# endernewton/tf-faster-rcnn

Hardware: NVIDIA H100
Metric: images/sec (higher is better)
Workload: dtype f16x3 (fp32-grade: fp16 hi/lo split of both operands, 3 wgmma f16 MMAs per product, fp32 accumulate)

## Files before the change

### include/frcnn_b200.h

```cpp
#ifndef FRCNN_B200_H_
#define FRCNN_B200_H_

#include <stddef.h>
#include <stdint.h>

#ifdef __cplusplus
extern "C" {
#endif

typedef enum {
  FRCNN_OK = 0,
  FRCNN_ERR_CUDA = -1,
  FRCNN_ERR_ARG = -2,
  FRCNN_ERR_NO_DEVICE = -3,
  FRCNN_ERR_DRIVER_ENTRY = -4,
  FRCNN_ERR_CAPACITY = -5
} frcnn_status;

#define FRCNN_NMS_PLUS_ONE 1u
#define FRCNN_NMS_INCLUSIVE 2u
#define FRCNN_NMS_SKIP_DEGENERATE 4u
#define FRCNN_NMS_MODE_CPU_NMS (FRCNN_NMS_PLUS_ONE | FRCNN_NMS_INCLUSIVE)
#define FRCNN_NMS_MODE_GPU_NMS (FRCNN_NMS_PLUS_ONE)
#define FRCNN_NMS_MODE_TF (FRCNN_NMS_SKIP_DEGENERATE)

#define FRCNN_ACT_NONE 0
#define FRCNN_ACT_RELU 1
#define FRCNN_ACT_RELU6 2

int frcnn_version(void);
int frcnn_last_error(char* buf, size_t buflen);
int frcnn_check_device(int device_id);
int frcnn_zero_async(void* dev_ptr, size_t bytes, void* stream);

typedef struct frcnn_graph frcnn_graph;
int frcnn_graph_begin(void* stream);
int frcnn_graph_end(void* stream, frcnn_graph** out);
int frcnn_graph_launch(const frcnn_graph* g, void* stream);
void frcnn_graph_destroy(frcnn_graph* g);

int frcnn_nms_host(int* keep_out, int* num_out, const float* boxes_host, int boxes_num, int boxes_dim,
                   float nms_overlap_thresh, int device_id, unsigned flags);

int frcnn_nms_sorted_dev(const float* boxes_dev, int n, float thresh, unsigned flags, int max_out,
                         int* keep_dev, int* num_dev, void* stream);

typedef struct frcnn_conv_plan frcnn_conv_plan;
#define FRCNN_CONV_F16X3 0
#define FRCNN_CONV_TF32X3 1
#define FRCNN_CONV_F16X1 2

typedef struct {
  const float* in_dev;
  const void* w_hi_dev;
  const void* w_lo_dev;
  const float* scale_dev;
  const float* shift_dev;
  const float* residual_dev;
  float* out_dev;
  int n, h, w, cin;
  int cout, kh, kw, stride;
  int pad_t, pad_l;
  int ho, wo;
  int act;
  int block_n;
  int kb_per_chunk;
  int split_k;
  int impl;
  float out_mult;
  const float* in2_dev;
  int cin2;
  float* mean_dev;
  int mean_hw;
} frcnn_conv_desc;

int frcnn_conv_plan_create(frcnn_conv_plan** out, const frcnn_conv_desc* d);
int frcnn_conv_plan_run(const frcnn_conv_plan* p, void* stream);
int frcnn_conv_plan_geometry(const frcnn_conv_desc* d, int sm_count, int* out16);
int frcnn_conv_plan_info(const frcnn_conv_plan* p, int* block_n, int* tile_n, int* tile_h, int* tile_w,
                         int* grid_m, int* grid_n, int* splits, int* smem_bytes);
int frcnn_conv_plan_set_trace(frcnn_conv_plan* p, long long* trace_dev);
void frcnn_conv_plan_destroy(frcnn_conv_plan* p);
int frcnn_debug_watchdog(unsigned int* out16, int reset);

int frcnn_pack_conv_weights(const float* w_hwio_dev, void* w_hi_dev, void* w_lo_dev, int kh, int kw,
                            int cin, int cout, int wexp, void* stream);
int frcnn_pack_conv_weights_tf32(const float* w_hwio_dev, float* w_hi_dev, float* w_lo_dev, int kh, int kw,
                                 int cin, int cout, void* stream);

int frcnn_conv_first(const float* in_dev, const float* w_hwio_dev, const float* scale_dev,
                     const float* shift_dev, float* out_dev, int n, int h, int w, int cout, int k,
                     int stride, int pad_t, int pad_l, int ho, int wo, int act, void* stream);
int frcnn_depthwise3x3(const float* in_dev, const float* w_dev, const float* scale_dev,
                       const float* shift_dev, float* out_dev, int n, int h, int w, int c, int stride,
                       int pad_t, int pad_l, int ho, int wo, int act, void* stream);
int frcnn_max_pool(const float* in_dev, float* out_dev, int n, int h, int w, int c, int k, int stride,
                   int pad_t, int pad_l, int ho, int wo, int pad_is_neg_inf, void* stream);
int frcnn_spatial_mean(const float* in_dev, float* out_dev, int r, int hw, int c, void* stream);

int frcnn_preprocess(const unsigned char* img_dev, int h0, int w0, const double* means3, double fx, double fy,
                     float* blob_dev, int H, int W, void* stream);
int frcnn_preprocess_hflip(const unsigned char* img_dev, int h0, int w0, const double* means3, double fx, double fy,
                           float* blob_dev, int H, int W, void* stream);


int frcnn_rpn_decode(const float* rpn_out_dev, int ld, int delta_col, const float* base_anchors_dev, int num_anchors,
                     int batch, int fh, int fw, int feat_stride, float im_h, float im_w, float* scores_dev,
                     float* props_dev, void* stream);
size_t frcnn_sort_workspace_bytes(int n);
int frcnn_sort_desc(const float* keys_dev, int n, int batch, int* order_dev, float* sorted_keys_dev, void* workspace_dev,
                    size_t workspace_bytes, void* stream);
int frcnn_proposals(const float* props_dev, const float* scores_dev, const int* order_dev, int n, int batch,
                    int pre_nms_top_n, int post_nms_top_n, float thresh, unsigned flags, float* rois_dev,
                    float* roi_scores_dev, int* keep_dev, int* num_dev, void* stream);
int frcnn_crop_pool(const float* feat_dev, int batch, int fh, int fw, int c, const float* rois_dev, int r, int pooled,
                    int pre_pool, float* out_dev, void* stream);
#define FRCNN_ROI_ALIGN_MAX_SAMPLING 16
int frcnn_roi_align(const float* feat_dev, int batch, int fh, int fw, int c, const float* rois_dev, int r, int pooled,
                    float spatial_scale, int sampling_ratio, int aligned, float* out_dev, void* stream);
int frcnn_roi_pool(const float* feat_dev, int batch, int fh, int fw, int c, const float* rois_dev, int r, int pooled,
                   float spatial_scale, float* out_dev, void* stream);
int frcnn_cls_finish(const float* head_out_dev, int ld, int r, int num_classes, const float* stds4,
                     const float* means4, float* cls_score_dev, float* cls_prob_dev, float* bbox_pred_dev,
                     void* stream);
int frcnn_bbox_decode(const float* rois_dev, const float* bbox_pred_dev, int r, int num_classes, int batch,
                      const float* im_meta_dev, float* pred_boxes_dev, void* stream);
size_t frcnn_detect_post_workspace_bytes(int r, int num_classes, int batch);
int frcnn_detect_post(const float* cls_prob_dev, const float* pred_boxes_dev, const int* num_rois_dev, int r, int batch,
                      int num_classes, float score_thresh, float nms_thresh, unsigned flags,
                      int max_per_image, int max_det, float* det_dev, int* ndet_dev, int record_stride, int* keep_dev,
                      int* keep_cnt_dev, float* keep_score_dev, void* workspace_dev, size_t workspace_bytes, void* stream);
#define FRCNN_SOFT_NMS_LINEAR 0
#define FRCNN_SOFT_NMS_GAUSSIAN 1
#define FRCNN_SOFT_NMS_HARD 2
int frcnn_soft_nms_host(float* dets_out, int* keep_out, int* num_out, const float* dets_host, int n, int dim, int method,
                        float sigma, float nt, float score_thresh, int device_id);
int frcnn_detect_post_soft(const float* cls_prob_dev, const float* pred_boxes_dev, const int* num_rois_dev, int r, int batch,
                           int num_classes, float score_thresh, int method, float sigma, float nt, float prune_thresh,
                           int max_per_image, int max_det, float* det_dev, int* ndet_dev, int record_stride, int* keep_dev,
                           int* keep_cnt_dev, float* keep_score_dev, void* workspace_dev, size_t workspace_bytes, void* stream);
#define FRCNN_BOX_VOTE_ID 0
#define FRCNN_BOX_VOTE_AVG 1
#define FRCNN_BOX_VOTE_IOU_AVG 2
#define FRCNN_BOX_VOTE_GENERALIZED_AVG 3
#define FRCNN_BOX_VOTE_QUASI_SUM 4
#define FRCNN_BOX_VOTE_TEMP_AVG 5
int frcnn_box_vote_host(float* dets_out, const float* top_host, int n_top, int top_dim, const float* all_host, int n_all,
                        int all_dim, float thresh, int method, float beta, int device_id);
int frcnn_detect_post_vote(const float* cls_prob_dev, const float* pred_boxes_dev, const int* num_rois_dev, int r, int batch,
                           int num_classes, float score_thresh, float nms_thresh, unsigned flags, int max_per_image, int max_det,
                           float* det_dev, int* ndet_dev, int record_stride, int* keep_dev, int* keep_cnt_dev, float* keep_score_dev,
                           void* workspace_dev, size_t workspace_bytes, float vote_thresh, int vote_method, float vote_beta,
                           float* vote_box_dev, void* stream);
int frcnn_detect_post_soft_vote(const float* cls_prob_dev, const float* pred_boxes_dev, const int* num_rois_dev, int r, int batch,
                                int num_classes, float score_thresh, int method, float sigma, float nt, float prune_thresh,
                                int max_per_image, int max_det, float* det_dev, int* ndet_dev, int record_stride, int* keep_dev,
                                int* keep_cnt_dev, float* keep_score_dev, void* workspace_dev, size_t workspace_bytes,
                                float vote_thresh, int vote_method, float vote_beta, float* vote_box_dev, void* stream);
int frcnn_detect_features(const int* keep_dev, const int* keep_cnt_dev, const float* fc7_dev, int r, int batch, int num_classes,
                          int feat_dim, int max_det, float* feat_out_dev, int* roi_out_dev, void* stream);
int frcnn_boxes_to_rois(const float* boxes_dev, const int* counts_dev, const float* im_meta_dev, int batch, int cap,
                        float* rois_dev, int* num_rois_dev, void* stream);

#define FRCNN_AUG_MAX_VIEWS 16
int frcnn_aug_union(const float* const* cls_prob_views, const float* const* pred_boxes_views, const int* const* num_rois_views,
                    const int* rois_per_view, const int* flip_views, int num_views, int batch, int num_classes,
                    const float* im_meta_dev, float* cls_prob_dev, float* pred_boxes_dev, int* num_rois_dev, void* stream);

#ifdef __cplusplus
}
#endif
#endif
// ... 1 lines not shown
```

### tf_faster_rcnn_b200/_native.py

```python
import ctypes as C
import os

_HERE = os.path.dirname(os.path.abspath(__file__))
LIB_PATH = os.path.join(_HERE, "libfrcnn_b200_wd.so" if os.environ.get("FRCNN_LIB_VARIANT") == "wd" else "libfrcnn_b200.so")

NMS_PLUS_ONE, NMS_INCLUSIVE, NMS_SKIP_DEGENERATE = 1, 2, 4
NMS_MODE_CPU_NMS = NMS_PLUS_ONE | NMS_INCLUSIVE
NMS_MODE_GPU_NMS = NMS_PLUS_ONE
NMS_MODE_TF = NMS_SKIP_DEGENERATE
ACT_NONE, ACT_RELU, ACT_RELU6 = 0, 1, 2
CONV_F16X3, CONV_TF32X3, CONV_F16X1 = 0, 1, 2
SOFT_NMS_METHODS = {"linear": 0, "gaussian": 1, "hard": 2}
AUG_MAX_VIEWS = 16
BOX_VOTE_METHODS = {"ID": 0, "AVG": 1, "IOU_AVG": 2, "GENERALIZED_AVG": 3, "QUASI_SUM": 4, "TEMP_AVG": 5}
ROI_ALIGN_MAX_SAMPLING = 16
ROI_MAX_POOLED = 16

vp, ci, cf, cu, sz = C.c_void_p, C.c_int, C.c_float, C.c_uint, C.c_size_t
ip, fp = C.POINTER(C.c_int), C.POINTER(C.c_float)


class ConvDesc(C.Structure):
    _fields_ = [("in_dev", vp), ("w_hi_dev", vp), ("w_lo_dev", vp), ("scale_dev", vp), ("shift_dev", vp),
                ("residual_dev", vp), ("out_dev", vp),
                ("n", ci), ("h", ci), ("w", ci), ("cin", ci), ("cout", ci), ("kh", ci), ("kw", ci), ("stride", ci),
                ("pad_t", ci), ("pad_l", ci), ("ho", ci), ("wo", ci), ("act", ci), ("block_n", ci), ("kb_per_chunk", ci), ("split_k", ci),
                ("impl", ci), ("out_mult", cf), ("in2_dev", vp), ("cin2", ci), ("mean_dev", vp), ("mean_hw", ci)]


SIGNATURES = {
    "frcnn_version": (ci, []),
    "frcnn_last_error": (ci, [C.c_char_p, sz]),
    "frcnn_check_device": (ci, [ci]),
    "frcnn_zero_async": (ci, [vp, sz, vp]),
    "frcnn_graph_begin": (ci, [vp]),
    "frcnn_graph_end": (ci, [vp, C.POINTER(vp)]),
    "frcnn_graph_launch": (ci, [vp, vp]),
    "frcnn_graph_destroy": (None, [vp]),
    "frcnn_nms_host": (ci, [ip, ip, fp, ci, ci, cf, ci, cu]),
    "frcnn_nms_sorted_dev": (ci, [vp, ci, cf, cu, ci, vp, vp, vp]),
    "frcnn_conv_plan_create": (ci, [C.POINTER(vp), C.POINTER(ConvDesc)]),
    "frcnn_conv_plan_run": (ci, [vp, vp]),
    "frcnn_conv_plan_geometry": (ci, [C.POINTER(ConvDesc), ci, ip]),
    "frcnn_conv_plan_info": (ci, [vp, ip, ip, ip, ip, ip, ip, ip, ip]),
    "frcnn_conv_plan_set_trace": (ci, [vp, vp]),
    "frcnn_conv_plan_destroy": (None, [vp]),
    "frcnn_debug_watchdog": (ci, [C.POINTER(C.c_uint), ci]),
    "frcnn_pack_conv_weights": (ci, [vp, vp, vp, ci, ci, ci, ci, ci, vp]),
    "frcnn_pack_conv_weights_tf32": (ci, [vp, vp, vp, ci, ci, ci, ci, vp]),
    "frcnn_conv_first": (ci, [vp, vp, vp, vp, vp, ci, ci, ci, ci, ci, ci, ci, ci, ci, ci, ci, vp]),
    "frcnn_depthwise3x3": (ci, [vp, vp, vp, vp, vp, ci, ci, ci, ci, ci, ci, ci, ci, ci, ci, vp]),
    "frcnn_max_pool": (ci, [vp, vp, ci, ci, ci, ci, ci, ci, ci, ci, ci, ci, ci, vp]),
    "frcnn_spatial_mean": (ci, [vp, vp, ci, ci, ci, vp]),
    "frcnn_preprocess": (ci, [vp, ci, ci, C.POINTER(C.c_double), C.c_double, C.c_double, vp, ci, ci, vp]),
    "frcnn_rpn_decode": (ci, [vp, ci, ci, vp, ci, ci, ci, ci, ci, cf, cf, vp, vp, vp]),
    "frcnn_sort_workspace_bytes": (sz, [ci]),
    "frcnn_sort_desc": (ci, [vp, ci, ci, vp, vp, vp, sz, vp]),
    "frcnn_proposals": (ci, [vp, vp, vp, ci, ci, ci, ci, cf, cu, vp, vp, vp, vp, vp]),
    "frcnn_crop_pool": (ci, [vp, ci, ci, ci, ci, vp, ci, ci, ci, vp, vp]),
    "frcnn_roi_align": (ci, [vp, ci, ci, ci, ci, vp, ci, ci, cf, ci, ci, vp, vp]),
    "frcnn_roi_pool": (ci, [vp, ci, ci, ci, ci, vp, ci, ci, cf, vp, vp]),
    "frcnn_cls_finish": (ci, [vp, ci, ci, ci, fp, fp, vp, vp, vp, vp]),
    "frcnn_bbox_decode": (ci, [vp, vp, ci, ci, ci, vp, vp, vp]),
    "frcnn_detect_post_workspace_bytes": (sz, [ci, ci, ci]),
    "frcnn_detect_post": (ci, [vp, vp, vp, ci, ci, ci, cf, cf, cu, ci, ci, vp, vp, ci, vp, vp, vp, vp, sz, vp]),
    "frcnn_soft_nms_host": (ci, [fp, ip, ip, fp, ci, ci, ci, cf, cf, cf, ci]),
    "frcnn_detect_post_soft": (ci, [vp, vp, vp, ci, ci, ci, cf, ci, cf, cf, cf, ci, ci, vp, vp, ci, vp, vp, vp, vp, sz, vp]),
    "frcnn_detect_features": (ci, [vp, vp, vp, ci, ci, ci, ci, ci, vp, vp, vp]),
    "frcnn_boxes_to_rois": (ci, [vp, vp, vp, ci, ci, vp, vp, vp]),
    "frcnn_preprocess_hflip": (ci, [vp, ci, ci, C.POINTER(C.c_double), C.c_double, C.c_double, vp, ci, ci, vp]),
    "frcnn_aug_union": (ci, [C.POINTER(vp), C.POINTER(vp), C.POINTER(vp), ip, ip, ci, ci, ci, vp, vp, vp, vp, vp]),
    "frcnn_box_vote_host": (ci, [fp, fp, ci, ci, fp, ci, ci, cf, ci, cf, ci]),
    "frcnn_detect_post_vote": (ci, [vp, vp, vp, ci, ci, ci, cf, cf, cu, ci, ci, vp, vp, ci, vp, vp, vp, vp, sz, cf, ci, cf, vp, vp]),
    "frcnn_detect_post_soft_vote": (ci, [vp, vp, vp, ci, ci, ci, cf, ci, cf, cf, cf, ci, ci, vp, vp, ci, vp, vp, vp, vp, sz, cf, ci, cf, vp,
                                         vp]),
}

_lib = None


def lib():
    global _lib
    if _lib is None:
        if not os.path.exists(LIB_PATH):
            raise RuntimeError("libfrcnn_b200.so not built (%s): the CUDA extension is mandatory, "
                               "there is no CPU fallback" % LIB_PATH)
        L = C.CDLL(LIB_PATH)
        for name, (res, args) in SIGNATURES.items():
            fn = getattr(L, name)
            fn.restype = res
            fn.argtypes = args
        _lib = L
    return _lib


def last_error():
    buf = C.create_string_buffer(512)
    lib().frcnn_last_error(buf, 512)
    return buf.value.decode("utf-8", "replace")


def check(rc, what=""):
    if rc != 0:
        raise RuntimeError("frcnn_b200 %s failed (status %d): %s" % (what, rc, last_error()))
```

### tf_faster_rcnn_b200/csrc/build.py

```python
import os
import subprocess
import sys
from concurrent.futures import ThreadPoolExecutor

HERE = os.path.dirname(os.path.abspath(__file__))
PKG = os.path.dirname(HERE)
SOURCES = ["api.cu", "conv_gemm.cu", "simt_ops.cu", "nms.cu", "sort.cu"]
HEADERS = ["common.cuh", os.path.join("..", "..", "include", "frcnn_b200.h")]
LIB = os.path.join(PKG, "libfrcnn_b200.so")
NVCC_FLAGS = ["-O3", "-std=c++17", "-lineinfo", "-gencode", "arch=compute_90a,code=sm_90a",
              "-Xcompiler", "-fPIC", "-Xptxas", "-v", "--expt-relaxed-constexpr"]


def _stale(dst, srcs):
    if not os.path.exists(dst):
        return True
    t = os.path.getmtime(dst)
    return any(os.path.getmtime(s) > t for s in srcs)


def build(force=False, verbose=False, watchdog=False):
    obj_dir = os.path.join(HERE, "_obj_wd" if watchdog else "_obj")
    lib = LIB.replace(".so", "_wd.so") if watchdog else LIB
    flags = NVCC_FLAGS + (["-DFRCNN_WATCHDOG"] if watchdog else [])
    os.makedirs(obj_dir, exist_ok=True)
    hdrs = [os.path.join(HERE, h) for h in HEADERS]
    jobs = []
    for s in SOURCES:
        src = os.path.join(HERE, s)
        obj = os.path.join(obj_dir, s.replace(".cu", ".o"))
        if force or _stale(obj, [src] + hdrs):
            jobs.append((src, obj))

    def cc(job):
        src, obj = job
        r = subprocess.run(["nvcc"] + flags + ["-c", src, "-o", obj], capture_output=True, text=True)
        log = r.stdout + r.stderr
        with open(obj + ".log", "w") as f:
            f.write(log)
        if r.returncode != 0:
            raise RuntimeError("nvcc failed for %s:\n%s" % (src, log))
        return log

    with ThreadPoolExecutor(max_workers=5) as ex:
        logs = list(ex.map(cc, jobs))
    if verbose:
        for l in logs:
            print(l)
    objs = [os.path.join(obj_dir, s.replace(".cu", ".o")) for s in SOURCES]
    if force or jobs or _stale(lib, objs):
        subprocess.check_call(["nvcc", "-shared", "-gencode", "arch=compute_90a,code=sm_90a", "-cudart", "static",
                               "-o", lib] + objs)
    return lib


if __name__ == "__main__":
    print(build(force="--force" in sys.argv, verbose=True, watchdog="--watchdog" in sys.argv))
```

### tf_faster_rcnn_b200/engine.py

```python
import collections
import ctypes
import os

import numpy as np
import torch

from . import _native as N
from . import ops

F = np.float32
C_void = ctypes.c_void_p


def bn_fold(gamma, beta, mean, var, eps):
    inv = (gamma.astype(F) * (F(1.0) / np.sqrt(var.astype(F) + F(eps)))).astype(F)
    return inv, (beta.astype(F) - mean.astype(F) * inv).astype(F)


def concat_layers(weights, names, bn_eps):
    ss = [weights.scale_shift(nm, bn_eps) for nm in names]
    w = ops.concat_scaled_weights([weights[nm + "/weights"] for nm in names], [s for s, _ in ss])
    shift = ss[0][1]
    for _, sh in ss[1:]:
        shift = (shift + sh).astype(F)
# ... 52 lines not shown
        if os.environ.get("FRCNN_TORCH_GRAPH") == "1":
            self._torch = torch.cuda.CUDAGraph()
            with torch.cuda.graph(self._torch):
                for fn in fns:
                    fn()
            return
        side = torch.cuda.Stream()
        side.wait_stream(torch.cuda.current_stream())
        with torch.cuda.stream(side):
            N.check(N.lib().frcnn_graph_begin(C_void(side.cuda_stream)), "graph_begin")
            try:
                for fn in fns:
                    fn()
            finally:
                rc = N.lib().frcnn_graph_end(C_void(side.cuda_stream), ctypes.byref(self._h))
            N.check(rc, "graph_end")
        torch.cuda.current_stream().wait_stream(side)

    def replay(self):
        if self._torch is not None:
            self._torch.replay()
        else:
            N.check(N.lib().frcnn_graph_launch(self._h, ops._stream()), "graph_launch")

    def __del__(self):
        try:
            if self._h:
                N.lib().frcnn_graph_destroy(self._h)
                self._h = ctypes.c_void_p()
        except Exception:
            pass


class Tape:
    def __init__(self, weights):
        self.w = weights
        self.steps = []
        self.flops = 0.0
        self.conv_flops = 0.0
        self.bufs = []
        self.conv_plans = []

    def new(self, *shape, dtype=torch.float32):
        t = torch.empty(shape, dtype=dtype, device="cuda")
        self.bufs.append(t)
        return t

    def add(self, label, fn):
        self.steps.append((label, fn))

    def run(self):
        for _, fn in self.steps:
            fn()

    def conv(self, x, name, stride=1, mode="SAME", act=N.ACT_RELU, bn_eps=None, residual=None, packed=None, x2=None, mean=False):
        pc = packed if packed is not None else self.w.packed_conv(name, bn_eps)
        n, h, w, _ = x.shape
        ho, wo, pt, pl = ops.conv_out_hw(h, w, pc.kh, stride, mode)
        out = self.new(n, pc.cout) if mean else self.new(n, ho, wo, pc.cout)
        plan = ops.ConvPlan(x, pc, out, stride, pt, pl, act, residual, x2=x2, mean=mean)
        self.conv_plans.append(plan)
        self.add("conv:" + name, plan.run)
        fl = 2.0 * n * ho * wo * pc.cout * pc.kh * pc.kw * pc.cin
        self.flops += fl
        self.conv_flops += fl
        return out

    def fc(self, x2d, name, act=N.ACT_NONE, packed=None):
        r, k = x2d.shape
        out = self.conv(x2d.view(1, 1, r, k), name, 1, "SAME", act, None, None, packed)
        return out.view(r, -1)

    def conv_first(self, x, name, k, stride, mode, act, bn_eps=None):
        sc, sh = self.w.scale_shift(name, bn_eps)
        wd = self.w.dev(name + "/weights", lambda: self.w[name + "/weights"])
        scd = None if sc is None else self.w.dev(name + "/scale", lambda: sc)
        shd = None if sh is None else self.w.dev(name + "/shift", lambda: sh)
        n, h, w, _ = x.shape
        ho, wo, pt, pl = ops.conv_out_hw(h, w, k, stride, mode)
        cout = int(self.w[name + "/weights"].shape[3])
        out = self.new(n, ho, wo, cout)
        self.add("conv_first:" + name, lambda: ops.conv_first(x, wd, scd, shd, out, k, stride, pt, pl, act))
        self.flops += 2.0 * n * ho * wo * cout * k * k * 3
        return out

    def depthwise(self, x, name, stride, act, bn_eps):
        sc, sh = self.w.scale_shift(name, bn_eps)
        c = x.shape[3]
        wd = self.w.dev(name + "/dw", lambda: self.w[name + "/depthwise_weights"].reshape(3, 3, c))
        scd = self.w.dev(name + "/scale", lambda: sc)
        shd = self.w.dev(name + "/shift", lambda: sh)
        n, h, w, _ = x.shape
        ho, wo, pt, pl = ops.conv_out_hw(h, w, 3, stride, "SAME" if stride == 1 else "EXPLICIT")
        out = self.new(n, ho, wo, c)
        self.add("depthwise:" + name, lambda: ops.depthwise3x3(x, wd, scd, shd, out, stride, pt, pl, act))
        return out

    def max_pool(self, x, k, stride, mode):
        n, h, w, c = x.shape
        if mode == "SAME":
            ho, wo = -(-h // stride), -(-w // stride)
            pt, _ = ops.same_pads(h, k, stride); pl, _ = ops.same_pads(w, k, stride)
            neg = True
        elif mode == "ZEROPAD1":
            ho, wo, pt, pl, neg = (h + 2 - k) // stride + 1, (w + 2 - k) // stride + 1, 1, 1, False
        else:
            ho, wo, pt, pl, neg = (h - k) // stride + 1, (w - k) // stride + 1, 0, 0, True
        out = self.new(n, ho, wo, c)
        self.add("max_pool", lambda: ops.max_pool(x, out, k, stride, pt, pl, neg))
        return out

    def spatial_mean(self, x):
        out = self.new(x.shape[0], x.shape[3])
        self.add("spatial_mean", lambda: ops.spatial_mean(x, out))
        return out


REC_HEADER = 8

PostKey = collections.namedtuple("PostKey", "score_thresh nms_thresh use_gpu_nms max_per_image soft_nms box_vote", defaults=(None,))


class PostStage:

    def __init__(self, net, batch, use_graph):
        self.net, self.batch = net, batch
        self.post_key = None
        self.recs = [None, None]
        self.rec = self.ndet = None
        self.post_steps = [None, None]
        self.feat_out = self.roi_out = self.features_step = None
        self.vote_box = None
        self.double_buffer = False
        self.slot = 0
        self.max_det = 0
        self.graphs = {}
        self.use_graph = use_graph

    def _ensure_post(self, features=False):
        o = self.net.options
        soft, vote = o.get("soft_nms"), o.get("box_vote")
        key = PostKey(float(o["score_thresh"]), float(o["nms_thresh"]), bool(o["use_gpu_nms"]), int(o["max_per_image"]),
                      None if soft is None else soft_nms_args(*soft), None if vote is None else box_vote_args(*vote))
        if key != self.post_key:
            self._build_post(key)
        if features and self.features_step is None:
            check_feature_mode(key.max_per_image)
            C, B, fdim = self.net.num_classes, self.batch, int(self.fc7.shape[1])
            self.feat_out = ops.zeros((B, self.max_det, fdim))
            self.roi_out = ops.zeros((B, self.max_det), dtype=torch.int32)
            self.features_step = lambda: ops.detect_features(self.keep, self.keep_cnt, self.fc7, C, self.feat_out, self.roi_out)

    def _build_post(self, key):
        C, R, B = self.net.num_classes, self.R, self.batch
        mpi, soft = key.max_per_image, key.soft_nms
        self.max_det = max_det = 2 * mpi + 56 if mpi > 0 else R * (C - 1)
        thr, flags = nms_threshold(key.nms_thresh, key.use_gpu_nms)
        self.vote_box = None if key.box_vote is None else ops.zeros((B, C, R, 4))
        vote = None if key.box_vote is None else (*key.box_vote, self.vote_box)

        def make_post(rec):
            det, ndet = rec.as_strided((B, max_det, 6), (rec.stride(0), 6, 1), REC_HEADER), rec.view(torch.int32)[:, 0]
            if soft is not None:
                return lambda: ops.detect_post_soft(self.cls_prob, self.pred_boxes, self.num_rois, C, key.score_thresh, soft[0], soft[1],
                                                    float(F(key.nms_thresh)), soft[2], mpi, det, ndet, self.keep, self.keep_cnt,
                                                    self.keep_score, batch=B, vote=vote)
# ... 431 lines not shown
```

### tf_faster_rcnn_b200/lib/nets/resnet_v1.py

```python
from nets.network import Network
from tf_faster_rcnn_b200 import _native as N

_UNITS = {50: (3, 4, 6, 3), 101: (3, 4, 23, 3), 152: (3, 8, 36, 3)}
_EPS = 1e-5


class resnetv1(Network):
    def __init__(self, num_layers=50):
        Network.__init__(self)
        if num_layers not in _UNITS:
            raise NotImplementedError
        self._num_layers = num_layers
        self._scope = 'resnet_v1_%d' % num_layers
        n1, n2, n3, n4 = _UNITS[num_layers]
        self._blocks = [("block1", 64, [1] * (n1 - 1) + [2]), ("block2", 128, [1] * (n2 - 1) + [2]),
                        ("block3", 256, [1] * n3), ("block4", 512, [1] * n4)]

    def crop_pre_pool(self):
        return bool(self.options["resnet_max_pool"])

    def _bottleneck(self, t, x, prefix, base, stride, mean=False):
        depth = 4 * base
        r = t.conv(x, prefix + "/conv1", 1, "SAME", N.ACT_RELU, _EPS)
        r = t.conv(r, prefix + "/conv2", stride, "SAME" if stride == 1 else "EXPLICIT", N.ACT_RELU, _EPS)
        if x.shape[3] == depth:
            shortcut = x if stride == 1 else t.max_pool(x, 1, stride, "VALID")
            return t.conv(r, prefix + "/conv3", 1, "SAME", N.ACT_RELU, _EPS, residual=shortcut, mean=mean)
        assert stride == 1
        pc = t.w.packed_concat([prefix + "/conv3", prefix + "/shortcut"], _EPS)
        return t.conv(r, prefix + "/conv3", 1, "SAME", N.ACT_RELU, packed=pc, x2=x, mean=mean)

    def _run_blocks(self, t, x, blocks, mean_last=False):
        for bi, (bname, base, strides) in enumerate(blocks):
            for u, s in enumerate(strides, start=1):
                last = bi == len(blocks) - 1 and u == len(strides)
                x = self._bottleneck(t, x, "%s/%s/unit_%d/bottleneck_v1" % (self._scope, bname, u), base, s, mean_last and last)
        return x

    def _image_to_head(self, t, image):
        x = t.conv_first(image, self._scope + "/conv1", 7, 2, "EXPLICIT", N.ACT_RELU, _EPS)
        x = t.max_pool(x, 3, 2, "ZEROPAD1")
        x = self._run_blocks(t, x, self._blocks[:3])
        self._layers['head'] = x
        return x

    def _head_to_tail(self, t, pool5):
        return self._run_blocks(t, pool5, self._blocks[3:], mean_last=True)
```

### tf_faster_rcnn_b200/ops.py

```python
import ctypes as C
import os

import numpy as np
import torch

from . import _native as N


def _stream():
    return C.c_void_p(torch.cuda.current_stream().cuda_stream)


def _p(t):
    return C.c_void_p(t.data_ptr()) if t is not None else C.c_void_p(0)


def _f32(t):
    assert t.dtype == torch.float32 and t.is_cuda and t.is_contiguous(), "expected contiguous cuda fp32"
    return t


def zeros(shape, dtype=torch.float32):
    t = torch.empty(shape, dtype=dtype, device="cuda")
    N.check(N.lib().frcnn_zero_async(_p(t), t.numel() * t.element_size(), _stream()), "zero_async")
# ... 33 lines not shown
            self.w_hi = torch.empty((self.cout, ktot), dtype=torch.float16, device="cuda")
            self.w_lo = torch.empty_like(self.w_hi)
            N.check(N.lib().frcnn_pack_conv_weights(_p(w), _p(self.w_hi), _p(self.w_lo), self.kh, self.kw, self.cin,
                                                    self.cout, self.wexp, _stream()), "pack_conv_weights")
        else:
            self.wexp, self.out_mult = 0, 1.0
            self.w_hi = torch.empty((self.cout, ktot), dtype=torch.float32, device="cuda")
            self.w_lo = torch.empty_like(self.w_hi)
            N.check(N.lib().frcnn_pack_conv_weights_tf32(_p(w), _p(self.w_hi), _p(self.w_lo), self.kh, self.kw, self.cin,
                                                         self.cout, _stream()), "pack_conv_weights_tf32")
        torch.cuda.current_stream().synchronize()
        self.scale = None if scale is None else torch.as_tensor(np.ascontiguousarray(scale), dtype=torch.float32).cuda()
        self.shift = None if shift is None else torch.as_tensor(np.ascontiguousarray(shift), dtype=torch.float32).cuda()


def concat_scaled_weights(ws, scales):
    parts = []
    for w, s in zip(ws, scales):
        w = np.asarray(w, dtype=np.float32)
        assert w.ndim == 4 and w.shape[:2] == (1, 1), w.shape
        parts.append(w if s is None else (w * np.asarray(s, dtype=np.float32)).astype(np.float32))
    return np.ascontiguousarray(np.concatenate(parts, axis=2))


class ConvPlan:

    def __init__(self, x, pc, out, stride=1, pad_t=0, pad_l=0, act=N.ACT_NONE, residual=None, block_n=0, kb_per_chunk=0, split_k=0,
                 x2=None, mean=False):
        _f32(x); _f32(out)
        n, h, w, cin = x.shape
        cin2 = 0
        if x2 is not None:
            _f32(x2)
            assert x2.shape[:3] == x.shape[:3], (x2.shape, x.shape)
            cin2 = int(x2.shape[3])
        assert cin + cin2 == pc.cin, (cin, cin2, pc.cin)
        if mean:
            ho, wo = h, w
            assert tuple(out.shape) == (n, pc.cout), (out.shape, n, pc.cout)
        else:
            no, ho, wo, co = out.shape
            assert no == n and co == pc.cout
        d = N.ConvDesc(_p(x), _p(pc.w_hi), _p(pc.w_lo), _p(pc.scale), _p(pc.shift), _p(residual), _p(None if mean else out),
                       n, h, w, cin, pc.cout, pc.kh, pc.kw, stride, pad_t, pad_l, ho, wo, act, block_n, kb_per_chunk, split_k,
                       pc.impl, pc.out_mult, _p(x2), cin2, _p(out if mean else None), h * w if mean else 0)
        self._h = C.c_void_p()
        N.check(N.lib().frcnn_conv_plan_create(C.byref(self._h), C.byref(d)), "conv_plan_create")
        self._keep = (x, pc, out, residual, x2)
        self.flops = 2.0 * n * ho * wo * pc.cout * pc.kh * pc.kw * pc.cin

    def run(self):
        N.check(N.lib().frcnn_conv_plan_run(self._h, _stream()), "conv_plan_run")

    def info(self):
        v = [C.c_int() for _ in range(8)]
        N.check(N.lib().frcnn_conv_plan_info(self._h, *[C.byref(a) for a in v]), "conv_plan_info")
        return dict(zip(["block_n", "tile_n", "tile_h", "tile_w", "grid_m", "grid_n", "splits", "smem"], [a.value for a in v]))

    def __del__(self):
        try:
            if self._h:
                N.lib().frcnn_conv_plan_destroy(self._h)
                self._h = C.c_void_p()
        except Exception:
            pass


def conv_out_hw(h, w, k, stride, mode):
    if mode == "SAME":
        pt, _ = same_pads(h, k, stride)
        pl, _ = same_pads(w, k, stride)
        return -(-h // stride), -(-w // stride), pt, pl
    pb = (k - 1) // 2
    return (h + k - 1 - k) // stride + 1, (w + k - 1 - k) // stride + 1, pb, pb


def conv_first(x, w_hwio_dev, scale, shift, out, k, stride, pad_t, pad_l, act):
    n, h, w, _ = x.shape
    _, ho, wo, co = out.shape
    N.check(N.lib().frcnn_conv_first(_p(_f32(x)), _p(w_hwio_dev), _p(scale), _p(shift), _p(_f32(out)), n, h, w, co, k, stride,
                                     pad_t, pad_l, ho, wo, act, _stream()), "conv_first")


def depthwise3x3(x, w_dev, scale, shift, out, stride, pad_t, pad_l, act):
    n, h, w, c = x.shape
    _, ho, wo, _ = out.shape
    N.check(N.lib().frcnn_depthwise3x3(_p(_f32(x)), _p(w_dev), _p(scale), _p(shift), _p(_f32(out)), n, h, w, c, stride, pad_t,
                                       pad_l, ho, wo, act, _stream()), "depthwise3x3")


def max_pool(x, out, k, stride, pad_t, pad_l, pad_is_neg_inf):
    n, h, w, c = x.shape
    _, ho, wo, _ = out.shape
    N.check(N.lib().frcnn_max_pool(_p(_f32(x)), _p(_f32(out)), n, h, w, c, k, stride, pad_t, pad_l, ho, wo,
                                   int(pad_is_neg_inf), _stream()), "max_pool")


def spatial_mean(x, out):
    r, hw, c = x.shape[0], x.shape[1] * x.shape[2], x.shape[3]
    N.check(N.lib().frcnn_spatial_mean(_p(_f32(x)), _p(_f32(out)), r, hw, c, _stream()), "spatial_mean")


def preprocess(img_u8_dev, means3, fx, fy, blob, hflip=False):
    h0, w0, _ = img_u8_dev.shape
    _, H, W, _ = blob.shape
    assert blob.is_contiguous()
    m = (C.c_double * 3)(*[float(v) for v in means3])
    fn = N.lib().frcnn_preprocess_hflip if hflip else N.lib().frcnn_preprocess
    N.check(fn(C.c_void_p(img_u8_dev.data_ptr()), h0, w0, m, float(fx), float(fy), _p(blob), H, W, _stream()),
            "preprocess_hflip" if hflip else "preprocess")


def rpn_decode(rpn_out, delta_col, base_anchors, num_anchors, fh, fw, im_h, im_w, scores, props, feat_stride=16, batch=1):
    ld = rpn_out.shape[-1]
    N.check(N.lib().frcnn_rpn_decode(_p(_f32(rpn_out)), ld, delta_col, _p(base_anchors), num_anchors, batch, fh, fw, feat_stride,
                                     float(im_h), float(im_w), _p(scores), _p(props), _stream()), "rpn_decode")


def sort_workspace(n):
    return torch.empty(int(N.lib().frcnn_sort_workspace_bytes(n)), dtype=torch.uint8, device="cuda")


def sort_desc(keys, order, sorted_keys, workspace=None, batch=1):
    n = keys.numel() // batch
    N.check(N.lib().frcnn_sort_desc(_p(_f32(keys)), n, batch, _p(order), _p(sorted_keys), _p(workspace),
                                    0 if workspace is None else workspace.numel(), _stream()), "sort_desc")


def proposals(props, scores, order, pre_nms_top_n, post_nms_top_n, thresh, flags, rois, roi_scores, keep, num, batch=1):
    n = scores.numel() // batch
    N.check(N.lib().frcnn_proposals(_p(props), _p(scores), _p(order), n, batch, pre_nms_top_n, post_nms_top_n, float(thresh), flags,
                                    _p(rois), _p(roi_scores), _p(keep), _p(num), _stream()), "proposals")


def crop_pool(feat, rois, pooled, pre_pool, out):
    b, fh, fw, c = feat.shape
    r = rois.shape[0]
    N.check(N.lib().frcnn_crop_pool(_p(_f32(feat)), b, fh, fw, c, _p(_f32(rois)), r, pooled, int(pre_pool), _p(_f32(out)), _stream()),
            "crop_pool")


def roi_align(feat, rois, pooled, spatial_scale, sampling_ratio, aligned, out):
    b, fh, fw, c = feat.shape
    N.check(N.lib().frcnn_roi_align(_p(_f32(feat)), b, fh, fw, c, _p(_f32(rois)), rois.shape[0], pooled, float(spatial_scale),
                                    int(sampling_ratio), int(bool(aligned)), _p(_f32(out)), _stream()), "roi_align")


def roi_pool(feat, rois, pooled, spatial_scale, out):
    b, fh, fw, c = feat.shape
    N.check(N.lib().frcnn_roi_pool(_p(_f32(feat)), b, fh, fw, c, _p(_f32(rois)), rois.shape[0], pooled, float(spatial_scale),
                                   _p(_f32(out)), _stream()), "roi_pool")


def cls_finish(head_out, num_classes, stds, means, cls_score, cls_prob, bbox_pred):
    r, ld = head_out.shape
    s4 = (C.c_float * 4)(*[float(v) for v in stds])
    m4 = (C.c_float * 4)(*[float(v) for v in means])
    N.check(N.lib().frcnn_cls_finish(_p(_f32(head_out)), ld, r, num_classes, s4, m4, _p(cls_score), _p(cls_prob), _p(bbox_pred),
                                     _stream()), "cls_finish")


def im_meta_tensor(rows):
    return torch.tensor([[float(np.float32(s)), float(h), float(w)] for s, h, w in rows], dtype=torch.float32).cuda()


def bbox_decode(rois, bbox_pred, num_classes, im_meta, pred_boxes):
# ... 107 lines not shown
```

Baseline: 260.2.

## Fuse ResNet stem 7x7 conv, BN/ReLU and 3x3 maxpool into one wgmma kernel

Adds a dedicated stem kernel that computes the 7x7 stride-2 conv with 3 input channels as a K=192 GEMM on wgmma, using an im2col-style tap table over an fp16 hi/lo input patch in shared memory. BN scale/shift and ReLU are applied in registers, and the 3x3/2 max pool runs from a shared-memory staging tile, so the full-resolution conv output never goes to global memory. The intent is to replace the SIMT conv_first plus a separate max_pool pass. In exchange it recomputes halo conv pixels at tile borders, and the tiles are small (121 rows of a 128-row MMA) with a synchronous wgmma wait per k-block.

```diff
diff --git a/include/frcnn_b200.h b/include/frcnn_b200.h
--- a/include/frcnn_b200.h
+++ b/include/frcnn_b200.h
@@ -88,6 +88,9 @@
 int frcnn_pack_conv_weights_tf32(const float* w_hwio_dev, float* w_hi_dev, float* w_lo_dev, int kh, int kw,
                                  int cin, int cout, void* stream);
 
+int frcnn_stem(const float* in_dev, const void* w_hi_dev, const void* w_lo_dev, const float* scale_dev, const float* shift_dev,
+               float out_mult, float* out_dev, int n, int h, int w, int cin, int cout, int impl, int conv_only, void* stream);
+
 int frcnn_conv_first(const float* in_dev, const float* w_hwio_dev, const float* scale_dev,
                      const float* shift_dev, float* out_dev, int n, int h, int w, int cout, int k,
                      int stride, int pad_t, int pad_l, int ho, int wo, int act, void* stream);
diff --git a/tf_faster_rcnn_b200/_native.py b/tf_faster_rcnn_b200/_native.py
--- a/tf_faster_rcnn_b200/_native.py
+++ b/tf_faster_rcnn_b200/_native.py
@@ -48,6 +48,7 @@
     "frcnn_debug_watchdog": (ci, [C.POINTER(C.c_uint), ci]),
     "frcnn_pack_conv_weights": (ci, [vp, vp, vp, ci, ci, ci, ci, ci, vp]),
     "frcnn_pack_conv_weights_tf32": (ci, [vp, vp, vp, ci, ci, ci, ci, vp]),
+    "frcnn_stem": (ci, [vp, vp, vp, vp, vp, cf, vp, ci, ci, ci, ci, ci, ci, ci, vp]),
     "frcnn_conv_first": (ci, [vp, vp, vp, vp, vp, ci, ci, ci, ci, ci, ci, ci, ci, ci, ci, ci, vp]),
     "frcnn_depthwise3x3": (ci, [vp, vp, vp, vp, vp, ci, ci, ci, ci, ci, ci, ci, ci, ci, ci, vp]),
     "frcnn_max_pool": (ci, [vp, vp, ci, ci, ci, ci, ci, ci, ci, ci, ci, ci, ci, vp]),
diff --git a/tf_faster_rcnn_b200/csrc/build.py b/tf_faster_rcnn_b200/csrc/build.py
--- a/tf_faster_rcnn_b200/csrc/build.py
+++ b/tf_faster_rcnn_b200/csrc/build.py
@@ -5,7 +5,7 @@
 
 HERE = os.path.dirname(os.path.abspath(__file__))
 PKG = os.path.dirname(HERE)
-SOURCES = ["api.cu", "conv_gemm.cu", "simt_ops.cu", "nms.cu", "sort.cu"]
+SOURCES = ["api.cu", "conv_gemm.cu", "stem.cu", "simt_ops.cu", "nms.cu", "sort.cu"]
 HEADERS = ["common.cuh", os.path.join("..", "..", "include", "frcnn_b200.h")]
 LIB = os.path.join(PKG, "libfrcnn_b200.so")
 NVCC_FLAGS = ["-O3", "-std=c++17", "-lineinfo", "-gencode", "arch=compute_90a,code=sm_90a",
diff --git a/tf_faster_rcnn_b200/csrc/stem.cu b/tf_faster_rcnn_b200/csrc/stem.cu
--- /dev/null
+++ b/tf_faster_rcnn_b200/csrc/stem.cu
@@ -0,0 +1,245 @@
+#include <cuda_fp16.h>
+#include "common.cuh"
+#include "../../include/frcnn_b200.h"
+
+namespace frcnn {
+namespace {
+
+constexpr int ST_PH = 5, ST_PW = 5;
+constexpr int ST_CH = 2 * ST_PH + 1, ST_CW = 2 * ST_PW + 1;
+constexpr int ST_PIX = ST_CH * ST_CW;
+constexpr int ST_IH = 2 * ST_CH + 6, ST_IW = 2 * ST_CW + 6;
+constexpr int ST_RS = ST_IW * 3;
+constexpr int ST_K = 192, ST_KB = 3, ST_COUT = 64;
+constexpr int ST_THREADS = 256;
+constexpr int ST_LD = ST_COUT + 8;
+constexpr int ST_W_PLANE = ST_KB * ST_COUT * 128;
+constexpr int ST_PATCH = ST_IH * ST_RS * 2;
+constexpr int ST_STAGE = ST_PIX * ST_LD * 4;
+constexpr int ST_TAB = ST_KB * 4 * 2;
+constexpr int ST_SMEM = 1024  + 2 * ST_W_PLANE + ST_STAGE + 2 * ST_PATCH + ST_TAB * 4 * 8 + 2 * ST_COUT * 4;
+constexpr int ST_PATCH_PAIRS = ST_IH * ST_RS / 2;
+constexpr int ST_PAIRS_PER_THREAD = (ST_PATCH_PAIRS + ST_THREADS - 1) / ST_THREADS;
+static_assert(ST_PIX <= 128, "the conv tile is one 128-row MMA tile");
+static_assert(ST_RS % 2 == 0, "fp16 pairs of the patch are 4-byte aligned");
+
+__device__ __forceinline__ void stem_tap(int k, int& r, int& s, int& c) {
+  const int tap = k / 12, ch = k % 12;
+  r = 2 * (tap >> 2) + ch / 6;
+  s = 2 * (tap & 3) + (ch % 6) / 3;
+  c = ch % 3;
+}
+
+__device__ __forceinline__ float stem_finish(float v, float sc, float sh) { return fmaxf(__fadd_rn(__fmul_rn(v, sc), sh), 0.f); }
+
+template <bool X1>
+__global__ void __launch_bounds__(ST_THREADS, 2)
+stem_kernel(const float* __restrict__ in, const __half* __restrict__ w_hi, const __half* __restrict__ w_lo,
+            const float* __restrict__ scale, const float* __restrict__ shift, float out_mult, float* __restrict__ out, int h, int w,
+            int ho, int wo, int hp, int wp, int tiles_x, int tiles_y, int ntiles, int conv_only) {
+  extern __shared__ uint8_t smem_raw[];
+  uint8_t* smem = reinterpret_cast<uint8_t*>((reinterpret_cast<uintptr_t>(smem_raw) + 1023) & ~uintptr_t(1023));
+  uint8_t* wsm = smem;
+  float* stage = reinterpret_cast<float*>(smem + 2 * ST_W_PLANE);
+  uint8_t* phi = reinterpret_cast<uint8_t*>(stage + ST_PIX * ST_LD);
+  uint8_t* plo = phi + ST_PATCH;
+  uint2* tab = reinterpret_cast<uint2*>(plo + ST_PATCH);
+  float* esc = reinterpret_cast<float*>(tab + ST_TAB * 4);
+  float* esh = esc + ST_COUT;
+  const int tid = threadIdx.x;
+
+  for (int i = tid; i < (X1 ? 1 : 2) * ST_KB * ST_COUT * 8; i += ST_THREADS) {
+    const int ch = i & 7, n = (i >> 3) & 63, kb = (i >> 9) % ST_KB, pl = (i >> 9) / ST_KB;
+    const __half* src = (pl ? w_lo : w_hi) + (size_t)n * ST_K + kb * 64 + ch * 8;
+    *reinterpret_cast<uint4*>(wsm + pl * ST_W_PLANE + kb * 8192 + n * 128 + ((ch ^ (n & 7)) << 4)) =
+        __ldg(reinterpret_cast<const uint4*>(src));
+  }
+  if (tid < ST_TAB * 4) {
+    const int q = tid >> 2, t = tid & 3;
+    const int k = (q >> 1) * 16 + (q & 1) * 8 + 2 * t;
+    int r, s0, c0, r1, s1, c1;
+    stem_tap(k, r, s0, c0);
+    stem_tap(k + 1, r1, s1, c1);
+    const uint32_t m = (r != 7 && s0 != 7 ? 0x0000ffffu : 0u) | (r1 != 7 && s1 != 7 ? 0xffff0000u : 0u);
+    tab[tid] = make_uint2((uint32_t)(2 * (r * ST_RS + 3 * s0 + c0)), m);
+  }
+  if (tid < ST_COUT) {
+    esc[tid] = __fmul_rn(scale ? scale[tid] : 1.f, out_mult);
+    esh[tid] = shift ? shift[tid] : 0.f;
+  }
+  asm volatile("fence.proxy.async.shared::cta;" ::: "memory");
+
+  const int warp = tid >> 5, lane = tid & 31, t4 = lane & 3;
+  const int row0 = (warp >> 2) * 64 + (warp & 3) * 16 + (lane >> 2);
+  uint32_t pbase[2];
+#pragma unroll
+  for (int e = 0; e < 2; ++e) {
+    const int m = min(row0 + 8 * e, ST_PIX - 1);
+    pbase[e] = (uint32_t)(2 * (2 * (m / ST_CW) * ST_RS + 6 * (m % ST_CW)));
+  }
+  const uint32_t w_a = smem_u32(wsm);
+
+  for (int tile = blockIdx.x; tile < ntiles; tile += gridDim.x) {
+    const int tx = tile % tiles_x, ty = (tile / tiles_x) % tiles_y, b = tile / (tiles_x * tiles_y);
+    const int py0 = ty * ST_PH, px0 = tx * ST_PW;
+    const int iy0 = 4 * py0 - 5, ix0 = 4 * px0 - 5;
+    float xs[ST_PAIRS_PER_THREAD][2];
+#pragma unroll
+    for (int u = 0; u < ST_PAIRS_PER_THREAD; ++u) {
+      const int i = tid + u * ST_THREADS;
+      const int row = i / (ST_RS / 2), f = 2 * (i % (ST_RS / 2));
+      const int iy = iy0 + row, g = ix0 * 3 + f;
+      xs[u][0] = xs[u][1] = 0.f;
+      if (i < ST_PATCH_PAIRS && iy >= 0 && iy < h) {
+        const float* src = in + ((size_t)b * h + iy) * w * 3;
+        if (g >= 0 && g < 3 * w) xs[u][0] = __ldg(src + g);
+        if (g + 1 >= 0 && g + 1 < 3 * w) xs[u][1] = __ldg(src + g + 1);
+      }
+    }
+    __syncthreads();
+#pragma unroll
+    for (int u = 0; u < ST_PAIRS_PER_THREAD; ++u) {
+      const int i = tid + u * ST_THREADS;
+      if (i < ST_PATCH_PAIRS) {
+        const int off = 2 * (i / (ST_RS / 2) * ST_RS + 2 * (i % (ST_RS / 2)));
+        const uint32_t hv = pack_f16x2_rn(xs[u][0], xs[u][1]);
+        *reinterpret_cast<uint32_t*>(phi + off) = hv;
+        if (!X1) {
+          const float2 fh = __half22float2(*reinterpret_cast<const __half2*>(&hv));
+          *reinterpret_cast<uint32_t*>(plo + off) =
+              pack_f16x2_rn(__fmul_rn(__fsub_rn(xs[u][0], fh.x), 2048.f), __fmul_rn(__fsub_rn(xs[u][1], fh.y), 2048.f));
+        }
+      }
+    }
+    __syncthreads();
+
+    float acc[32], part[32];
+#pragma unroll
+    for (int i = 0; i < 32; ++i) { acc[i] = 0.f; part[i] = 0.f; }
+#pragma unroll 1
+    for (int kb = 0; kb < ST_KB; ++kb) {
+      uint32_t ahi[4][4], alo[4][4];
+#pragma unroll
+      for (int j = 0; j < 4; ++j)
+#pragma unroll
+        for (int hf = 0; hf < 2; ++hf) {
+          const uint2 te = tab[((kb * 4 + j) * 2 + hf) * 4 + t4];
+#pragma unroll
+          for (int e = 0; e < 2; ++e) {
+            ahi[j][hf * 2 + e] = *reinterpret_cast<const uint32_t*>(phi + pbase[e] + te.x) & te.y;
+            alo[j][hf * 2 + e] = X1 ? 0u : *reinterpret_cast<const uint32_t*>(plo + pbase[e] + te.x) & te.y;
+          }
+        }
+      const uint64_t bhi = wgmma_sw128_desc(w_a + (uint32_t)(kb * 8192));
+      const uint64_t blo = wgmma_sw128_desc(w_a + (uint32_t)(ST_W_PLANE + kb * 8192));
+#pragma unroll
+      for (int i = 0; i < 32; ++i) reg_fence(part[i]);
+      wgmma_fence();
+#pragma unroll
+      for (int j = 0; j < 4; ++j) wgmma_f16_rs<64>(part, ahi[j], bhi + 2u * j, j > 0 ? 1u : 0u);
+      wgmma_commit();
+      wgmma_wait_all();
+#pragma unroll
+      for (int i = 0; i < 32; ++i) { reg_fence(part[i]); acc[i] = __fadd_rn(acc[i], part[i]); }
+      if (!X1) {
+        wgmma_fence();
+#pragma unroll
+        for (int j = 0; j < 4; ++j) {
+          wgmma_f16_rs<64>(part, alo[j], bhi + 2u * j, j > 0 ? 1u : 0u);
+          wgmma_f16_rs<64>(part, ahi[j], blo + 2u * j, 1u);
+        }
+        wgmma_commit();
+        wgmma_wait_all();
+#pragma unroll
+        for (int i = 0; i < 32; ++i) { reg_fence(part[i]); acc[i] = __fmaf_rn(part[i], 0.00048828125f, acc[i]); }
+      }
+    }
+
+#pragma unroll
+    for (int e = 0; e < 2; ++e) {
+      const int m = row0 + 8 * e;
+      if (m >= ST_PIX) continue;
+      const int ly = m / ST_CW, lx = m % ST_CW;
+      const int cy = 2 * py0 - 1 + ly, cx = 2 * px0 - 1 + lx;
+      const bool inside = cy >= 0 && cy < ho && cx >= 0 && cx < wo;
+      if (conv_only) {
+        if (!inside || ly == 0 || lx == 0 || ly > 2 * ST_PH || lx > 2 * ST_PW) continue;
+        float* o = out + (((size_t)b * ho + cy) * wo + cx) * ST_COUT;
+#pragma unroll
+        for (int j = 0; j < 8; ++j) {
+          const int c = 8 * j + 2 * t4;
+          *reinterpret_cast<float2*>(o + c) = make_float2(stem_finish(acc[4 * j + 2 * e], esc[c], esh[c]),
+                                                          stem_finish(acc[4 * j + 2 * e + 1], esc[c + 1], esh[c + 1]));
+        }
+      } else {
+        float* s = stage + m * ST_LD;
+#pragma unroll
+        for (int j = 0; j < 8; ++j) {
+          const int c = 8 * j + 2 * t4;
+          *reinterpret_cast<float2*>(s + c) =
+              inside ? make_float2(stem_finish(acc[4 * j + 2 * e], esc[c], esh[c]), stem_finish(acc[4 * j + 2 * e + 1], esc[c + 1], esh[c + 1]))
+                     : make_float2(0.f, 0.f);
+        }
+      }
+    }
+    if (conv_only) continue;
+    __syncthreads();
+    for (int i = tid; i < ST_PH * ST_PW * (ST_COUT / 4); i += ST_THREADS) {
+      const int cg = i % (ST_COUT / 4), q = i / (ST_COUT / 4), qy = q / ST_PW, qx = q % ST_PW;
+      const int py = py0 + qy, px = px0 + qx;
+      if (py >= hp || px >= wp) continue;
+      const float ninf = __int_as_float(0xff800000);
+      float4 mx = make_float4(ninf, ninf, ninf, ninf);
+#pragma unroll
+      for (int r = 0; r < 3; ++r)
+#pragma unroll
+        for (int s = 0; s < 3; ++s) {
+          const float4 v = *reinterpret_cast<const float4*>(stage + ((2 * qy + r) * ST_CW + 2 * qx + s) * ST_LD + 4 * cg);
+          mx.x = fmaxf(mx.x, v.x); mx.y = fmaxf(mx.y, v.y); mx.z = fmaxf(mx.z, v.z); mx.w = fmaxf(mx.w, v.w);
+        }
+      *reinterpret_cast<float4*>(out + (((size_t)b * hp + py) * wp + px) * ST_COUT + 4 * cg) = mx;
+    }
+  }
+}
+
+template <bool X1>
+int stem_launch(const float* in, const void* w_hi, const void* w_lo, const float* scale, const float* shift, float out_mult, float* out,
+                int n, int h, int w, int conv_only, cudaStream_t st) {
+  static int max_grid = 0;
+  if (max_grid == 0) {
+    FRCNN_CUDA(cudaFuncSetAttribute(stem_kernel<X1>, cudaFuncAttributeMaxDynamicSharedMemorySize, ST_SMEM));
+    int dev = 0, sms = 0, per_sm = 0;
+    FRCNN_CUDA(cudaGetDevice(&dev));
+    FRCNN_CUDA(cudaDeviceGetAttribute(&sms, cudaDevAttrMultiProcessorCount, dev));
+    FRCNN_CUDA(cudaOccupancyMaxActiveBlocksPerMultiprocessor(&per_sm, stem_kernel<X1>, ST_THREADS, ST_SMEM));
+    FRCNN_REQUIRE(per_sm > 0, "stem: the kernel does not fit on an SM");
+    max_grid = sms * per_sm;
+  }
+  const int ho = (h - 1) / 2 + 1, wo = (w - 1) / 2 + 1;
+  const int hp = (ho - 1) / 2 + 1, wp = (wo - 1) / 2 + 1;
+  const int tiles_x = cdiv(wp, ST_PW), tiles_y = cdiv(hp, ST_PH);
+  const long ntiles = (long)tiles_x * tiles_y * n;
+  FRCNN_REQUIRE(ntiles < (1l << 31), "stem: %ld tiles", ntiles);
+  const int grid = (int)(ntiles < max_grid ? ntiles : max_grid);
+  stem_kernel<X1><<<grid, ST_THREADS, ST_SMEM, st>>>(in, (const __half*)w_hi, (const __half*)w_lo, scale, shift, out_mult, out, h, w,
+                                                     ho, wo, hp, wp, tiles_x, tiles_y, (int)ntiles, conv_only);
+  FRCNN_LAUNCH_CHECK();
+  return OK;
+}
+
+}
+}
+
+using namespace frcnn;
+
+extern "C" int frcnn_stem(const float* in_dev, const void* w_hi_dev, const void* w_lo_dev, const float* scale_dev, const float* shift_dev,
+                          float out_mult, float* out_dev, int n, int h, int w, int cin, int cout, int impl, int conv_only, void* stream) {
+  FRCNN_REQUIRE(cin == 3 && cout == 64, "stem: cin must be 3 and cout 64 (got %d, %d)", cin, cout);
+  FRCNN_REQUIRE(impl == FRCNN_CONV_F16X3 || impl == FRCNN_CONV_F16X1, "stem: impl %d: only FRCNN_CONV_F16X3 and FRCNN_CONV_F16X1", impl);
+  FRCNN_REQUIRE(in_dev && w_hi_dev && out_dev && (w_lo_dev || impl == FRCNN_CONV_F16X1), "stem: null pointer");
+  FRCNN_REQUIRE(n > 0 && h > 0 && w > 0, "stem: bad shape %d x %d x %d", n, h, w);
+  FRCNN_REQUIRE(out_mult > 0.f, "stem: out_mult must be 2^-wexp of the packed weights");
+  if (impl == FRCNN_CONV_F16X1)
+    return stem_launch<true>(in_dev, w_hi_dev, w_lo_dev, scale_dev, shift_dev, out_mult, out_dev, n, h, w, conv_only, (cudaStream_t)stream);
+  return stem_launch<false>(in_dev, w_hi_dev, w_lo_dev, scale_dev, shift_dev, out_mult, out_dev, n, h, w, conv_only, (cudaStream_t)stream);
+}
diff --git a/tf_faster_rcnn_b200/engine.py b/tf_faster_rcnn_b200/engine.py
--- a/tf_faster_rcnn_b200/engine.py
+++ b/tf_faster_rcnn_b200/engine.py
@@ -158,6 +158,18 @@
         out = self.new(n, ho, wo, cout)
         self.add("conv_first:" + name, lambda: ops.conv_first(x, wd, scd, shd, out, k, stride, pt, pl, act))
         self.flops += 2.0 * n * ho * wo * cout * k * k * 3
+        return out
+
+    def stem(self, x, name, bn_eps):
+        if ops.conv_impl() == N.CONV_TF32X3:
+            return self.max_pool(self.conv_first(x, name, 7, 2, "EXPLICIT", N.ACT_RELU, bn_eps), 3, 2, "ZEROPAD1")
+        pc = self.w.packed_custom(name + "/stem",
+                                  lambda: (ops.stem_weights(self.w[name + "/weights"]),) + self.w.scale_shift(name, bn_eps))
+        n, h, w, _ = x.shape
+        ho, wo, hp, wp = ops.stem_out_hw(h, w)
+        out = self.new(n, hp, wp, pc.cout)
+        self.add("stem:" + name, lambda: ops.stem(x, pc, out))
+        self.flops += 2.0 * n * ho * wo * pc.cout * 7 * 7 * 3
         return out
 
     def depthwise(self, x, name, stride, act, bn_eps):
diff --git a/tf_faster_rcnn_b200/lib/nets/resnet_v1.py b/tf_faster_rcnn_b200/lib/nets/resnet_v1.py
--- a/tf_faster_rcnn_b200/lib/nets/resnet_v1.py
+++ b/tf_faster_rcnn_b200/lib/nets/resnet_v1.py
@@ -38,8 +38,7 @@
         return x
 
     def _image_to_head(self, t, image):
-        x = t.conv_first(image, self._scope + "/conv1", 7, 2, "EXPLICIT", N.ACT_RELU, _EPS)
-        x = t.max_pool(x, 3, 2, "ZEROPAD1")
+        x = t.stem(image, self._scope + "/conv1", _EPS)
         x = self._run_blocks(t, x, self._blocks[:3])
         self._layers['head'] = x
         return x
diff --git a/tf_faster_rcnn_b200/ops.py b/tf_faster_rcnn_b200/ops.py
--- a/tf_faster_rcnn_b200/ops.py
+++ b/tf_faster_rcnn_b200/ops.py
@@ -139,6 +139,35 @@
                                      pad_t, pad_l, ho, wo, act, _stream()), "conv_first")
 
 
+def stem_k_table():
+    k = np.arange(192)
+    tap, ch = k // 12, k % 12
+    return np.stack([2 * (tap // 4) + ch // 6, 2 * (tap % 4) + (ch % 6) // 3, ch % 3], axis=1)
+
+
+def stem_weights(w_hwio):
+    w = np.asarray(w_hwio, dtype=np.float32)
+    assert w.shape[:3] == (7, 7, 3), w.shape
+    w8 = np.zeros((8, 8, 3, w.shape[3]), np.float32)
+    w8[:7, :7] = w
+    t = stem_k_table()
+    return np.ascontiguousarray(w8[t[:, 0], t[:, 1], t[:, 2]].reshape(4, 4, 12, w.shape[3]))
+
+
+def stem_out_hw(h, w):
+    ho, wo = (h - 1) // 2 + 1, (w - 1) // 2 + 1
+    return ho, wo, (ho - 1) // 2 + 1, (wo - 1) // 2 + 1
+
+
+def stem(x, pc, out, conv_only=False):
+    n, h, w, cin = x.shape
+    ho, wo, hp, wp = stem_out_hw(h, w)
+    assert (pc.kh, pc.kw, pc.cin) == (4, 4, 12), "pc must pack stem_weights(w)"
+    assert tuple(out.shape) == ((n, ho, wo, pc.cout) if conv_only else (n, hp, wp, pc.cout)), out.shape
+    N.check(N.lib().frcnn_stem(_p(_f32(x)), _p(pc.w_hi), _p(pc.w_lo), _p(pc.scale), _p(pc.shift), pc.out_mult, _p(_f32(out)), n, h, w,
+                               cin, pc.cout, pc.impl, int(bool(conv_only)), _stream()), "stem")
+
+
 def depthwise3x3(x, w_dev, scale, shift, out, stride, pad_t, pad_l, act):
     n, h, w, c = x.shape
     _, ho, wo, _ = out.shape
```

Result: faster. 265.2 (median of 6 runs) (+1.9%).
